# pearl-robot-lab/2HandedAfforder

Measured on AMD Instinct MI355X. Metric: affordance frames/sec/GPU @1024^2, 32-tok prompt; mask IoU vs ref, higher is better.
Workload: dtype bf16

## Files before the change

2handedafforder_amd/csrc/window_attention.hip:

```cpp
#include "haff_common.h"

namespace {

struct WinArgs {
  const bf16_t *q, *k, *v;
  bf16_t* o;
  long q_sb, q_sh, q_st;
  long k_sb, k_sh, k_st;
  long v_sb, v_sh, v_st;
  long o_sb, o_sh, o_st;
  int B, H;
  float scale;
  const bf16_t *tab_h, *tab_w;
  int grid_h, grid_w, wps;
  long pad_token;
};

constexpr float WLOG2E = 1.4426950408889634f;
typedef __attribute__((address_space(3))) bf16x4* wlds_v4_ptr;
typedef const __attribute__((address_space(1))) void* wgptr_t;
typedef __attribute__((address_space(3))) void* wlptr_t;
__device__ __attribute__((aligned(16))) unsigned int haff_win_zero_page[4];

template <int D, int S>
struct WinCfg {
  static constexpr int N = S * S;
  static constexpr int NKD = (D + 31) / 32;
  static constexpr int ND = D / 16;
  static constexpr int CPR = D / 8;
  static constexpr int KPC = (D * 2) % 64 == 32 ? 0 : 2;
  static constexpr int KSTR = D * 2 + 16 * KPC;
  static constexpr int VSTR = D * 2;
  static constexpr int NKS = (S + 1) / 2;
  static constexpr int RS = 52;
  static constexpr int QPW = 2;
  static constexpr int NWAVES = (S + QPW - 1) / QPW;
  static constexpr int NTHREADS = 64 * NWAVES;
  static constexpr int KSLOTS = N * (CPR + KPC), VSLOTS = N * CPR;
  static constexpr int K_BYTES = N * KSTR, V_BYTES = N * VSTR;
  static constexpr int PAD_SLOTS = (KSLOTS + VSLOTS + 63) / 64 * 64;
  static constexpr int BUF_BYTES = PAD_SLOTS * 16;
  static constexpr int SC_BYTES = NWAVES * 16 * RS * 4;
  static constexpr int LDS_BYTES = 2 * BUF_BYTES + SC_BYTES;
};

template <int D, int S, bool F16 = false>
__global__ __launch_bounds__((WinCfg<D, S>::NTHREADS)) void window_attn_kernel(WinArgs p) {
  using E = h16<F16>;
  using C = WinCfg<D, S>;
  static_assert(D % 16 == 0 && D <= 96 && S <= 16 && 2 * S - 1 <= 32, "window kernel geometry");
  extern __shared__ __attribute__((aligned(16))) unsigned char wsm[];
  float* sScr = reinterpret_cast<float*>(wsm + 2 * C::BUF_BYTES);

  const int tid = threadIdx.x;
  const int lane = tid & 63;
  const int wave = __builtin_amdgcn_readfirstlane(tid >> 6);
  const int fr = lane & 15, fh = lane >> 4;
  const int n_items = p.B * p.H;

  auto decode = [&](int id, int& win, int& h) {
    if ((p.B & 7) == 0) {
      const int x = id & 7, kseq = id >> 3;
      win = (kseq / p.H) * 8 + x;
      h = kseq - (kseq / p.H) * p.H;
    } else {
      win = id / p.H;
      h = id - win * p.H;
    }
  };

  constexpr int TOTAL_SLOTS = C::KSLOTS + C::VSLOTS;
  constexpr int NDMA = (C::PAD_SLOTS + C::NTHREADS - 1) / C::NTHREADS;
  static_assert((C::K_BYTES % 16) == 0 && C::KSTR == (C::CPR + C::KPC) * 16 && C::VSTR == C::CPR * 16 && C::KSTR % 64 == 32, "slot layout");
  unsigned slot_off[NDMA];
  unsigned slot_pad[NDMA];
  const long v_minus_k = (p.v - p.k);
  const unsigned vmk_bytes = (unsigned)(v_minus_k * 2);
#pragma unroll
  for (int i = 0; i < NDMA; ++i) {
    const int sl = tid + i * C::NTHREADS;
    long off;
    unsigned pad = 0;
    if (sl >= TOTAL_SLOTS) {
      off = 0;
    } else if (sl < C::KSLOTS) {
      const int row = sl / (C::CPR + C::KPC), c = sl - row * (C::CPR + C::KPC);
      off = (long)row * p.k_st + (c < C::CPR ? c * 8 : 0);
      pad = ((unsigned)(row / S) << 28) | ((unsigned)(row % S) << 24) | (unsigned)((c < C::CPR ? c : 0) * 16);
    } else {
      const int sv = sl - C::KSLOTS;
      const int row = sv / C::CPR, c = sv - row * C::CPR;
      off = v_minus_k + (long)row * p.v_st + c * 8;
      pad = ((unsigned)(row / S) << 28) | ((unsigned)(row % S) << 24) | (1u << 23) | (unsigned)(c * 16);
    }
    slot_off[i] = (unsigned)(off * 2);
    slot_pad[i] = pad;
  }
  uint4 qnext[C::QPW][C::NKD];
  const int qcol = min(fr, S - 1);
  const bf16_t* nx_kb = p.k;
  int nx_pad_h0 = S, nx_pad_w0 = S;
  unsigned nx_pad_base = 0, nx_lds0 = 0;
  auto begin_loads = [&](int id, int buf) {
    int win, h;
    decode(id, win, h);
    const bf16_t* qb = p.q + (long)win * p.q_sb + (long)h * p.q_sh;
    const bf16_t* kb = p.k + (long)win * p.k_sb + (long)h * p.k_sh;
    int pad_h0 = S, pad_w0 = S;
    if (p.grid_h > 0) {
      const int wi = win % (p.wps * p.wps);
      pad_h0 = p.grid_h - (wi / p.wps) * S;
      pad_w0 = p.grid_w - (wi % p.wps) * S;
    }
    const unsigned pad_base = (unsigned)((p.pad_token * p.k_st - (long)win * p.k_sb) * 2);
    const bf16_t* qpad = p.q + p.pad_token * p.q_st + (long)h * p.q_sh;
#pragma unroll
    for (int t = 0; t < C::QPW; ++t) {
      const int qh_t = min(wave + t * C::NWAVES, S - 1);
      const bf16_t* qsrc = (qh_t >= pad_h0 || qcol >= pad_w0) ? qpad : qb + (long)(qh_t * S + qcol) * p.q_st;
#pragma unroll
      for (int kd = 0; kd < C::NKD; ++kd) {
        const int col = kd * 32 + fh * 8;
        qnext[t][kd] = make_uint4(0, 0, 0, 0);
        if (col < D) qnext[t][kd] = *reinterpret_cast<const uint4*>(qsrc + col);
      }
    }
    nx_kb = kb;
    nx_pad_h0 = pad_h0;
    nx_pad_w0 = pad_w0;
    nx_pad_base = pad_base;
    nx_lds0 = (unsigned)(uintptr_t)(wlptr_t)(wsm + buf * C::BUF_BYTES) + wave * 1024;
  };
  auto issue_dma = [&](int i0, int i1) {
#pragma unroll
    for (int i = 0; i < NDMA; ++i) {
      if (i < i0 || i >= i1) continue;
      const unsigned m0v = nx_lds0 + i * C::NTHREADS * 16;
      const bool is_pad = (int)(slot_pad[i] >> 28) >= nx_pad_h0 || (int)((slot_pad[i] >> 24) & 15u) >= nx_pad_w0;
      const unsigned off = is_pad ? nx_pad_base + (slot_pad[i] & 0xffu) + ((slot_pad[i] >> 23) & 1u) * vmk_bytes : slot_off[i];
      if ((i + 1) * C::NTHREADS <= C::PAD_SLOTS || (i * C::NTHREADS + wave * 64) < C::PAD_SLOTS)
        asm volatile("s_mov_b32 m0, %2\n\ts_nop 0\n\tglobal_load_lds_dwordx4 %0, %1" ::"v"(off), "s"(nx_kb), "s"(m0v)
                     : "memory");
    }
  };
  constexpr int DMA_Q1 = (NDMA + 3) / 4, DMA_Q2 = (NDMA + 1) / 2, DMA_Q3 = (3 * NDMA + 3) / 4;

  auto settle_q = [&]() {
#pragma unroll
    for (int t = 0; t < C::QPW; ++t)
#pragma unroll
      for (int kd = 0; kd < C::NKD; ++kd)
        asm volatile("" : "+v"(qnext[t][kd].x), "+v"(qnext[t][kd].y), "+v"(qnext[t][kd].z), "+v"(qnext[t][kd].w));
  };

  int item = blockIdx.x;
  if (item >= n_items) return;
  begin_loads(item, 0);
  issue_dma(0, NDMA);

  bf16x8 th[2][C::NKD], tw[2][C::NKD];
#pragma unroll
  for (int mt = 0; mt < 2; ++mt) {
    const int r = min(mt * 16 + fr, 2 * S - 2);
#pragma unroll
    for (int kd = 0; kd < C::NKD; ++kd) {
      const int col = kd * 32 + fh * 8;
      uint4 a = make_uint4(0, 0, 0, 0), b = make_uint4(0, 0, 0, 0);
      if (col < D) {
        a = *reinterpret_cast<const uint4*>(p.tab_h + r * D + col);
        b = *reinterpret_cast<const uint4*>(p.tab_w + r * D + col);
      }
      th[mt][kd] = __builtin_bit_cast(bf16x8, a);
      tw[mt][kd] = __builtin_bit_cast(bf16x8, b);
    }
  }
  asm volatile("s_waitcnt vmcnt(0)" ::: "memory");
  settle_q();
#pragma unroll
  for (int mt = 0; mt < 2; ++mt)
#pragma unroll
    for (int kd = 0; kd < C::NKD; ++kd) {
      asm volatile("" : "+v"(th[mt][kd]));
      asm volatile("" : "+v"(tw[mt][kd]));
    }
  __syncthreads();

  const float sl2 = p.scale * WLOG2E;
  float* scr = sScr + wave * (16 * C::RS);
  const int tr_q = fr >> 2, tr_p = fr & 3;
  bool kw_ok[4];
#pragma unroll
  for (int j = 0; j < 4; ++j) kw_ok[j] = (4 * fh + j) < S;

  for (int it = 0;; ++it) {
    const int buf = it & 1;
    const unsigned char* sK = wsm + buf * C::BUF_BYTES;
    const unsigned char* sV = sK + C::K_BYTES;
    int win, h;
    decode(item, win, h);
    bf16_t* ob = p.o + (long)win * p.o_sb + (long)h * p.o_sh;
    uint4 qcur[C::QPW][C::NKD];
#pragma unroll
    for (int t = 0; t < C::QPW; ++t)
#pragma unroll
      for (int kd = 0; kd < C::NKD; ++kd) qcur[t][kd] = qnext[t][kd];
    const int next = item + gridDim.x;
    const bool has_next = next < n_items;
    if (has_next) {
      begin_loads(next, buf ^ 1);
      issue_dma(0, DMA_Q1);
    }

#pragma unroll
    for (int t = 0; t < C::QPW; ++t) {
      const int qh = wave + t * C::NWAVES;
      static_assert(C::QPW * C::NWAVES == S, "q-tiles must divide evenly over the waves");
      bf16x8 qraw[C::NKD], qs[C::NKD];
#pragma unroll
      for (int kd = 0; kd < C::NKD; ++kd) {
        const uint4 r = qcur[t][kd];
        uint4 rs = make_uint4(0, 0, 0, 0);
        if (kd * 32 + fh * 8 < D) {
          float qv[8];
          const unsigned w4[4] = {r.x, r.y, r.z, r.w};
#pragma unroll
          for (int j = 0; j < 4; ++j) {
            qv[2 * j] = E::lo(w4[j]) * sl2;
            qv[2 * j + 1] = E::hi(w4[j]) * sl2;
          }
          rs.x = E::pack2(qv[0], qv[1]); rs.y = E::pack2(qv[2], qv[3]);
          rs.z = E::pack2(qv[4], qv[5]); rs.w = E::pack2(qv[6], qv[7]);
        }
        qraw[kd] = __builtin_bit_cast(bf16x8, r);
        qs[kd] = __builtin_bit_cast(bf16x8, rs);
      }

      float relw4[4], relh_t[S];
      {
        f32x4 t0 = f32x4{0.f, 0.f, 0.f, 0.f}, t1 = t0;
#pragma unroll
        for (int kd = 0; kd < C::NKD; ++kd) {
          t0 = E::mfma16(tw[0][kd], qraw[kd], t0);
          t1 = E::mfma16(tw[1][kd], qraw[kd], t1);
        }
        float a[4] = {t0[0], t0[1], t0[2], t0[3]}, b[4] = {t1[0], t1[1], t1[2], t1[3]};
        store4(scr + fr * C::RS + 4 * fh, a);
        store4(scr + fr * C::RS + 16 + 4 * fh, b);
        __builtin_amdgcn_wave_barrier();
#pragma unroll
        for (int j = 0; j < 4; ++j) {
          const int r = min(max(qcol - (4 * fh + j) + S - 1, 0), 2 * S - 2);
          relw4[j] = kw_ok[j] ? scr[fr * C::RS + r] * WLOG2E : -INFINITY;
        }
        __builtin_amdgcn_wave_barrier();
      }
      {
        f32x4 t0 = f32x4{0.f, 0.f, 0.f, 0.f}, t1 = t0;
#pragma unroll
        for (int kd = 0; kd < C::NKD; ++kd) {
          t0 = E::mfma16(th[0][kd], qraw[kd], t0);
          t1 = E::mfma16(th[1][kd], qraw[kd], t1);
        }
        float a[4] = {t0[0], t0[1], t0[2], t0[3]}, b[4] = {t1[0], t1[1], t1[2], t1[3]};
        store4(scr + fr * C::RS + 4 * fh, a);
        store4(scr + fr * C::RS + 16 + 4 * fh, b);
        __builtin_amdgcn_wave_barrier();
#pragma unroll
        for (int kt = 0; kt < S; ++kt) relh_t[kt] = scr[fr * C::RS + (qh - kt + S - 1)] * WLOG2E;
        __builtin_amdgcn_wave_barrier();
      }

      f32x4 sacc[S];
#pragma unroll
      for (int kt = 0; kt < S; ++kt)
        sacc[kt] = f32x4{relw4[0] + relh_t[kt], relw4[1] + relh_t[kt], relw4[2] + relh_t[kt], relw4[3] + relh_t[kt]};
      constexpr int KG = (S + 1) / 2;
      const int koff_last = (D * 2 - (C::NKD - 1) * 64 == 32) ? (C::NKD - 1) * 64 - 32 + ((fh + 2) & 3) * 16
                                                              : min(fh * 16 + (C::NKD - 1) * 64, D * 2 - 16);
#pragma unroll
      for (int g0 = 0; g0 < S; g0 += KG) {
#pragma unroll
        for (int kd = 0; kd < C::NKD; ++kd) {
#pragma unroll
          for (int kt = g0; kt < g0 + KG && kt < S; ++kt) {
            const bf16x8 kf = *reinterpret_cast<const bf16x8*>(sK + (kt * S + qcol) * C::KSTR + (kd == C::NKD - 1 ? koff_last : fh * 16 + kd * 64));
            sacc[kt] = E::mfma16(kf, qs[kd], sacc[kt]);
          }
        }
        __builtin_amdgcn_sched_barrier(0);
      }

      if (has_next) {
        if (t == 0) issue_dma(DMA_Q1, DMA_Q2);
        else issue_dma(DMA_Q3, NDMA);
      }
      float mx = -1e30f;
#pragma unroll
      for (int kt = 0; kt < S; ++kt)
#pragma unroll
        for (int j = 0; j < 4; ++j) mx = fmaxf(mx, sacc[kt][j]);
      mx = fmaxf(mx, __shfl_xor(mx, 16, 64));
      mx = fmaxf(mx, __shfl_xor(mx, 32, 64));
      float psum = 0.f;
#pragma unroll
      for (int kt = 0; kt < S; ++kt)
#pragma unroll
        for (int j = 0; j < 4; ++j) {
          const float e = __builtin_amdgcn_exp2f(sacc[kt][j] - mx);
          sacc[kt][j] = e;
          psum += e;
        }
      psum += __shfl_xor(psum, 16, 64);
      psum += __shfl_xor(psum, 32, 64);

      f32x4 oacc[C::ND];
#pragma unroll
      for (int dt = 0; dt < C::ND; ++dt) oacc[dt] = f32x4{0.f, 0.f, 0.f, 0.f};
      const int vkw = min(4 * fh + tr_q, S - 1);
#pragma unroll
      for (int ks = 0; ks < C::NKS; ++ks) {
        constexpr int dummy = 0; (void)dummy;
        const int t0 = 2 * ks, t1 = (2 * ks + 1 < S) ? 2 * ks + 1 : 2 * ks;
        uint4 u;
        u.x = E::pack2(sacc[t0][0], sacc[t0][1]);
        u.y = E::pack2(sacc[t0][2], sacc[t0][3]);
        u.z = (2 * ks + 1 < S) ? E::pack2(sacc[t1][0], sacc[t1][1]) : 0u;
        u.w = (2 * ks + 1 < S) ? E::pack2(sacc[t1][2], sacc[t1][3]) : 0u;
        const bf16x8 pf = __builtin_bit_cast(bf16x8, u);
        const unsigned char* v0 = sV + (t0 * S + vkw) * C::VSTR + 8 * tr_p;
        const unsigned char* v1 = sV + (t1 * S + vkw) * C::VSTR + 8 * tr_p;
#pragma unroll
        for (int dt = 0; dt < C::ND; ++dt) {
          const bf16x4 lo = __builtin_amdgcn_ds_read_tr16_b64_v4i16((wlds_v4_ptr)(v0 + 32 * dt));
          const bf16x4 hi = __builtin_amdgcn_ds_read_tr16_b64_v4i16((wlds_v4_ptr)(v1 + 32 * dt));
          const bf16x8 vf = __builtin_shufflevector(lo, hi, 0, 1, 2, 3, 4, 5, 6, 7);
          oacc[dt] = E::mfma16(vf, pf, oacc[dt]);
        }
      }

      if (has_next && t == 0) issue_dma(DMA_Q2, DMA_Q3);
      const float inv = 1.0f / psum;
      if (fr < S) {
        bf16_t* orow = ob + (long)(qh * S + fr) * p.o_st + 4 * fh;
#pragma unroll
        for (int dt = 0; dt < C::ND; ++dt) {
          float v[4] = {oacc[dt][0] * inv, oacc[dt][1] * inv, oacc[dt][2] * inv, oacc[dt][3] * inv};
          store4h<F16>(orow + 16 * dt, v);
        }
      }
    }

    if (!has_next) break;
    item = next;
    asm volatile("s_waitcnt vmcnt(0)" ::: "memory");
    settle_q();
    __syncthreads();
  }
}

}

template <bool F16 = false>
static int window_attention_impl(const void* q, long q_sb, long q_sh, long q_st,
                                 const void* k, long k_sb, long k_sh, long k_st,
                                 const void* v, long v_sb, long v_sh, long v_st,
                                 void* o, long o_sb, long o_sh, long o_st,
                                 int n_windows, int H, int S, int d, float scale,
                                 const void* tab_h, const void* tab_w, int grid_h, int grid_w,
                                 long pad_token, void* stream) {
  if (n_windows <= 0 || H <= 0 || S <= 0 || d <= 0 || !tab_h || !tab_w) return HAFF_ERR_BAD_ARG;
  if ((q_st & 7) || (k_st & 7) || (v_st & 7) || (o_st & 3) || (q_sh & 7) || (k_sh & 7) || (v_sh & 7) || (o_sh & 3) ||
      (q_sb & 7) || (k_sb & 7) || (v_sb & 7) || (o_sb & 3))
    return HAFF_ERR_BAD_ARG;
  if ((reinterpret_cast<uintptr_t>(q) & 15) || (reinterpret_cast<uintptr_t>(k) & 15) ||
      (reinterpret_cast<uintptr_t>(v) & 15) || (reinterpret_cast<uintptr_t>(o) & 7) ||
      (reinterpret_cast<uintptr_t>(tab_h) & 15) || (reinterpret_cast<uintptr_t>(tab_w) & 15))
    return HAFF_ERR_BAD_ARG;
  if (S != 14 || d != 80) return HAFF_ERR_UNSUPPORTED;
  if (k_sb != v_sb || k_sh != v_sh || k_st != v_st) return HAFF_ERR_UNSUPPORTED;
  {
    const long dvk = reinterpret_cast<const bf16_t*>(v) - reinterpret_cast<const bf16_t*>(k);
    const long span = (dvk < 0 ? -dvk : dvk) + (long)S * S * k_st + d;
    if (dvk < 0 || span * 2 >= (1L << 32)) return HAFF_ERR_UNSUPPORTED;
  }
  WinArgs p{reinterpret_cast<const bf16_t*>(q), reinterpret_cast<const bf16_t*>(k), reinterpret_cast<const bf16_t*>(v),
            reinterpret_cast<bf16_t*>(o), q_sb, q_sh, q_st, k_sb, k_sh, k_st, v_sb, v_sh, v_st, o_sb, o_sh, o_st,
            n_windows, H, scale, reinterpret_cast<const bf16_t*>(tab_h), reinterpret_cast<const bf16_t*>(tab_w),
            grid_h, grid_w, grid_h > 0 ? (grid_h + S - 1) / S : 0, pad_token};
  if (grid_h > 0) {
    if (grid_w != grid_h || (n_windows % (p.wps * p.wps)) != 0 || pad_token < 0 || q_st != k_st ||
        (pad_token + 1) * k_st * 2 >= (1L << 32) || pad_token * k_st < (long)(n_windows - 1) * k_sb)
      return HAFF_ERR_BAD_ARG;
    const long dvk = reinterpret_cast<const bf16_t*>(v) - reinterpret_cast<const bf16_t*>(k);
    if ((pad_token * k_st + dvk + d) * 2 >= (1L << 32)) return HAFF_ERR_UNSUPPORTED;
  }
  using C = WinCfg<80, 14>;
  if (hipFuncSetAttribute(reinterpret_cast<const void*>(&window_attn_kernel<80, 14, F16>),
                          hipFuncAttributeMaxDynamicSharedMemorySize, C::LDS_BYTES) != hipSuccess)
    return HAFF_ERR_LAUNCH;
  const int n_items = n_windows * H;
  dim3 grid(n_items < 256 ? n_items : 256), block(C::NTHREADS);
  hipLaunchKernelGGL((window_attn_kernel<80, 14, F16>), grid, block, C::LDS_BYTES, reinterpret_cast<hipStream_t>(stream), p);
  return haff_check_launch();
}

extern "C" int haff_window_attention_bf16(const void* q, long q_sb, long q_sh, long q_st,
                                          const void* k, long k_sb, long k_sh, long k_st,
                                          const void* v, long v_sb, long v_sh, long v_st,
                                          void* o, long o_sb, long o_sh, long o_st,
                                          int n_windows, int H, int S, int d, float scale,
                                          const void* tab_h, const void* tab_w, int grid_h, int grid_w,
                                          long pad_token, void* stream) {
  return window_attention_impl(q, q_sb, q_sh, q_st, k, k_sb, k_sh, k_st, v, v_sb, v_sh, v_st, o, o_sb, o_sh, o_st, n_windows, H, S,
                               d, scale, tab_h, tab_w, grid_h, grid_w, pad_token, stream);
}

extern "C" int haff_window_attention_f16(const void* q, long q_sb, long q_sh, long q_st,
                                         const void* k, long k_sb, long k_sh, long k_st,
                                         const void* v, long v_sb, long v_sh, long v_st,
                                         void* o, long o_sb, long o_sh, long o_st,
                                         int n_windows, int H, int S, int d, float scale,
                                         const void* tab_h, const void* tab_w, int grid_h, int grid_w,
                                         long pad_token, void* stream) {
  return window_attention_impl<true>(q, q_sb, q_sh, q_st, k, k_sb, k_sh, k_st, v, v_sb, v_sh, v_st, o, o_sb, o_sh, o_st, n_windows, H,
                                     S, d, scale, tab_h, tab_w, grid_h, grid_w, pad_token, stream);
}
```

Baseline: 114.1.

## Interleave both query tiles per wave and move rel-pos tables to LDS

Processes both query rows of each wave together, so every K and V LDS fragment read is reused across two MFMAs and one rel-pos table fragment feeds both tiles. The relative-position tables move from per-thread registers into LDS, written once by wave 0. Slot pad metadata is now recomputed only for edge windows instead of being kept in registers, and the Q prefetch is deferred to after softmax. The aim is lower register pressure and fewer LDS reads per MFMA, at the cost of larger live accumulator arrays (two sets of sacc and oacc), extra LDS reads for the table fragments, and a different DMA issue schedule.

```diff
diff --git a/2handedafforder_amd/csrc/window_attention.hip b/2handedafforder_amd/csrc/window_attention.hip
--- a/2handedafforder_amd/csrc/window_attention.hip
+++ b/2handedafforder_amd/csrc/window_attention.hip
@@ -41,7 +41,8 @@
   static constexpr int PAD_SLOTS = (KSLOTS + VSLOTS + 63) / 64 * 64;
   static constexpr int BUF_BYTES = PAD_SLOTS * 16;
   static constexpr int SC_BYTES = NWAVES * 16 * RS * 4;
-  static constexpr int LDS_BYTES = 2 * BUF_BYTES + SC_BYTES;
+  static constexpr int TAB_BYTES = 2 * 2 * NKD * 64 * 16;
+  static constexpr int LDS_BYTES = 2 * BUF_BYTES + SC_BYTES + TAB_BYTES;
 };
 
 template <int D, int S, bool F16 = false>
@@ -51,6 +52,7 @@
   static_assert(D % 16 == 0 && D <= 96 && S <= 16 && 2 * S - 1 <= 32, "window kernel geometry");
   extern __shared__ __attribute__((aligned(16))) unsigned char wsm[];
   float* sScr = reinterpret_cast<float*>(wsm + 2 * C::BUF_BYTES);
+  unsigned char* sTab = wsm + 2 * C::BUF_BYTES + C::SC_BYTES;
 
   const int tid = threadIdx.x;
   const int lane = tid & 63;
@@ -72,33 +74,37 @@
   constexpr int TOTAL_SLOTS = C::KSLOTS + C::VSLOTS;
   constexpr int NDMA = (C::PAD_SLOTS + C::NTHREADS - 1) / C::NTHREADS;
   static_assert((C::K_BYTES % 16) == 0 && C::KSTR == (C::CPR + C::KPC) * 16 && C::VSTR == C::CPR * 16 && C::KSTR % 64 == 32, "slot layout");
-  unsigned slot_off[NDMA];
-  unsigned slot_pad[NDMA];
   const long v_minus_k = (p.v - p.k);
   const unsigned vmk_bytes = (unsigned)(v_minus_k * 2);
+  auto slot_pad = [&](int sl) -> unsigned {
+    if (sl >= TOTAL_SLOTS) return 0u;
+    if (sl < C::KSLOTS) {
+      const int row = sl / (C::CPR + C::KPC), c = sl - row * (C::CPR + C::KPC);
+      return ((unsigned)(row / S) << 28) | ((unsigned)(row % S) << 24) | (unsigned)((c < C::CPR ? c : 0) * 16);
+    }
+    const int sv = sl - C::KSLOTS;
+    const int row = sv / C::CPR, c = sv - row * C::CPR;
+    return ((unsigned)(row / S) << 28) | ((unsigned)(row % S) << 24) | (1u << 23) | (unsigned)(c * 16);
+  };
+  unsigned slot_off[NDMA];
 #pragma unroll
   for (int i = 0; i < NDMA; ++i) {
     const int sl = tid + i * C::NTHREADS;
-    long off;
-    unsigned pad = 0;
-    if (sl >= TOTAL_SLOTS) {
-      off = 0;
-    } else if (sl < C::KSLOTS) {
+    long off = 0;
+    if (sl < C::KSLOTS) {
       const int row = sl / (C::CPR + C::KPC), c = sl - row * (C::CPR + C::KPC);
       off = (long)row * p.k_st + (c < C::CPR ? c * 8 : 0);
-      pad = ((unsigned)(row / S) << 28) | ((unsigned)(row % S) << 24) | (unsigned)((c < C::CPR ? c : 0) * 16);
-    } else {
+    } else if (sl < TOTAL_SLOTS) {
       const int sv = sl - C::KSLOTS;
       const int row = sv / C::CPR, c = sv - row * C::CPR;
       off = v_minus_k + (long)row * p.v_st + c * 8;
-      pad = ((unsigned)(row / S) << 28) | ((unsigned)(row % S) << 24) | (1u << 23) | (unsigned)(c * 16);
     }
     slot_off[i] = (unsigned)(off * 2);
-    slot_pad[i] = pad;
   }
   uint4 qnext[C::QPW][C::NKD];
   const int qcol = min(fr, S - 1);
   const bf16_t* nx_kb = p.k;
+  const bf16_t* nx_q[C::QPW];
   int nx_pad_h0 = S, nx_pad_w0 = S;
   unsigned nx_pad_base = 0, nx_lds0 = 0;
   auto begin_loads = [&](int id, int buf) {
@@ -117,13 +123,7 @@
 #pragma unroll
     for (int t = 0; t < C::QPW; ++t) {
       const int qh_t = min(wave + t * C::NWAVES, S - 1);
-      const bf16_t* qsrc = (qh_t >= pad_h0 || qcol >= pad_w0) ? qpad : qb + (long)(qh_t * S + qcol) * p.q_st;
-#pragma unroll
-      for (int kd = 0; kd < C::NKD; ++kd) {
-        const int col = kd * 32 + fh * 8;
-        qnext[t][kd] = make_uint4(0, 0, 0, 0);
-        if (col < D) qnext[t][kd] = *reinterpret_cast<const uint4*>(qsrc + col);
-      }
+      nx_q[t] = (qh_t >= pad_h0 || qcol >= pad_w0) ? qpad : qb + (long)(qh_t * S + qcol) * p.q_st;
     }
     nx_kb = kb;
     nx_pad_h0 = pad_h0;
@@ -131,13 +131,26 @@
     nx_pad_base = pad_base;
     nx_lds0 = (unsigned)(uintptr_t)(wlptr_t)(wsm + buf * C::BUF_BYTES) + wave * 1024;
   };
+  auto load_q = [&]() {
+#pragma unroll
+    for (int t = 0; t < C::QPW; ++t)
+#pragma unroll
+      for (int kd = 0; kd < C::NKD; ++kd)
+        qnext[t][kd] = *reinterpret_cast<const uint4*>(nx_q[t] + min(kd * 32 + fh * 8, D - 8));
+  };
   auto issue_dma = [&](int i0, int i1) {
 #pragma unroll
     for (int i = 0; i < NDMA; ++i) {
       if (i < i0 || i >= i1) continue;
       const unsigned m0v = nx_lds0 + i * C::NTHREADS * 16;
-      const bool is_pad = (int)(slot_pad[i] >> 28) >= nx_pad_h0 || (int)((slot_pad[i] >> 24) & 15u) >= nx_pad_w0;
-      const unsigned off = is_pad ? nx_pad_base + (slot_pad[i] & 0xffu) + ((slot_pad[i] >> 23) & 1u) * vmk_bytes : slot_off[i];
+      unsigned off = slot_off[i];
+      if (nx_pad_h0 < S || nx_pad_w0 < S) {
+        int t_id = tid;
+        asm volatile("" : "+v"(t_id));
+        const unsigned sp = slot_pad(t_id + i * C::NTHREADS);
+        if ((int)(sp >> 28) >= nx_pad_h0 || (int)((sp >> 24) & 15u) >= nx_pad_w0)
+          off = nx_pad_base + (sp & 0xffu) + ((sp >> 23) & 1u) * vmk_bytes;
+      }
       if ((i + 1) * C::NTHREADS <= C::PAD_SLOTS || (i * C::NTHREADS + wave * 64) < C::PAD_SLOTS)
         asm volatile("s_mov_b32 m0, %2\n\ts_nop 0\n\tglobal_load_lds_dwordx4 %0, %1" ::"v"(off), "s"(nx_kb), "s"(m0v)
                      : "memory");
@@ -156,33 +169,40 @@
   int item = blockIdx.x;
   if (item >= n_items) return;
   begin_loads(item, 0);
+  load_q();
   issue_dma(0, NDMA);
 
-  bf16x8 th[2][C::NKD], tw[2][C::NKD];
-#pragma unroll
-  for (int mt = 0; mt < 2; ++mt) {
-    const int r = min(mt * 16 + fr, 2 * S - 2);
-#pragma unroll
-    for (int kd = 0; kd < C::NKD; ++kd) {
-      const int col = kd * 32 + fh * 8;
-      uint4 a = make_uint4(0, 0, 0, 0), b = make_uint4(0, 0, 0, 0);
-      if (col < D) {
-        a = *reinterpret_cast<const uint4*>(p.tab_h + r * D + col);
-        b = *reinterpret_cast<const uint4*>(p.tab_w + r * D + col);
-      }
-      th[mt][kd] = __builtin_bit_cast(bf16x8, a);
-      tw[mt][kd] = __builtin_bit_cast(bf16x8, b);
-    }
+  auto tab_frag = [&](int tab, int mt, int kd) -> unsigned char* {
+    return sTab + ((tab * 2 + mt) * C::NKD + kd) * 1024 + lane * 16;
+  };
+  if (wave == 0) {
+    uint4 tv[2][2][C::NKD];
+#pragma unroll
+    for (int mt = 0; mt < 2; ++mt) {
+      const int r = min(mt * 16 + fr, 2 * S - 2);
+#pragma unroll
+      for (int kd = 0; kd < C::NKD; ++kd) {
+        const int col = kd * 32 + fh * 8;
+        tv[0][mt][kd] = tv[1][mt][kd] = make_uint4(0, 0, 0, 0);
+        if (col < D) {
+          tv[0][mt][kd] = *reinterpret_cast<const uint4*>(p.tab_h + r * D + col);
+          tv[1][mt][kd] = *reinterpret_cast<const uint4*>(p.tab_w + r * D + col);
+        }
+      }
+    }
+    asm volatile("s_waitcnt vmcnt(0)" ::: "memory");
+#pragma unroll
+    for (int tb = 0; tb < 2; ++tb)
+#pragma unroll
+      for (int mt = 0; mt < 2; ++mt)
+#pragma unroll
+        for (int kd = 0; kd < C::NKD; ++kd) {
+          asm volatile("" : "+v"(tv[tb][mt][kd].x), "+v"(tv[tb][mt][kd].y), "+v"(tv[tb][mt][kd].z), "+v"(tv[tb][mt][kd].w));
+          *reinterpret_cast<uint4*>(tab_frag(tb, mt, kd)) = tv[tb][mt][kd];
+        }
   }
   asm volatile("s_waitcnt vmcnt(0)" ::: "memory");
   settle_q();
-#pragma unroll
-  for (int mt = 0; mt < 2; ++mt)
-#pragma unroll
-    for (int kd = 0; kd < C::NKD; ++kd) {
-      asm volatile("" : "+v"(th[mt][kd]));
-      asm volatile("" : "+v"(tw[mt][kd]));
-    }
   __syncthreads();
 
   const float sl2 = p.scale * WLOG2E;
@@ -199,6 +219,7 @@
     int win, h;
     decode(item, win, h);
     bf16_t* ob = p.o + (long)win * p.o_sb + (long)h * p.o_sh;
+    settle_q();
     uint4 qcur[C::QPW][C::NKD];
 #pragma unroll
     for (int t = 0; t < C::QPW; ++t)
@@ -211,16 +232,17 @@
       issue_dma(0, DMA_Q1);
     }
 
-#pragma unroll
-    for (int t = 0; t < C::QPW; ++t) {
-      const int qh = wave + t * C::NWAVES;
-      static_assert(C::QPW * C::NWAVES == S, "q-tiles must divide evenly over the waves");
-      bf16x8 qraw[C::NKD], qs[C::NKD];
+    static_assert(C::QPW * C::NWAVES == S, "q-tiles must divide evenly over the waves");
+    constexpr int T = C::QPW;
+    bf16x8 qraw[T][C::NKD], qs[T][C::NKD];
+#pragma unroll
+    for (int t = 0; t < T; ++t)
 #pragma unroll
       for (int kd = 0; kd < C::NKD; ++kd) {
-        const uint4 r = qcur[t][kd];
+        const bool in_d = kd * 32 + fh * 8 < D;
+        const uint4 r = in_d ? qcur[t][kd] : make_uint4(0, 0, 0, 0);
         uint4 rs = make_uint4(0, 0, 0, 0);
-        if (kd * 32 + fh * 8 < D) {
+        if (in_d) {
           float qv[8];
           const unsigned w4[4] = {r.x, r.y, r.z, r.w};
 #pragma unroll
@@ -231,120 +253,140 @@
           rs.x = E::pack2(qv[0], qv[1]); rs.y = E::pack2(qv[2], qv[3]);
           rs.z = E::pack2(qv[4], qv[5]); rs.w = E::pack2(qv[6], qv[7]);
         }
-        qraw[kd] = __builtin_bit_cast(bf16x8, r);
-        qs[kd] = __builtin_bit_cast(bf16x8, rs);
-      }
-
-      float relw4[4], relh_t[S];
-      {
-        f32x4 t0 = f32x4{0.f, 0.f, 0.f, 0.f}, t1 = t0;
-#pragma unroll
-        for (int kd = 0; kd < C::NKD; ++kd) {
-          t0 = E::mfma16(tw[0][kd], qraw[kd], t0);
-          t1 = E::mfma16(tw[1][kd], qraw[kd], t1);
-        }
-        float a[4] = {t0[0], t0[1], t0[2], t0[3]}, b[4] = {t1[0], t1[1], t1[2], t1[3]};
+        qraw[t][kd] = __builtin_bit_cast(bf16x8, r);
+        qs[t][kd] = __builtin_bit_cast(bf16x8, rs);
+      }
+
+    float relw4[T][4], relh_t[T][S];
+#pragma unroll
+    for (int tb = 1; tb >= 0; --tb) {
+      f32x4 ta[T][2];
+#pragma unroll
+      for (int t = 0; t < T; ++t) ta[t][0] = ta[t][1] = f32x4{0.f, 0.f, 0.f, 0.f};
+#pragma unroll
+      for (int kd = 0; kd < C::NKD; ++kd) {
+        const bf16x8 f0 = *reinterpret_cast<const bf16x8*>(tab_frag(tb, 0, kd));
+        const bf16x8 f1 = *reinterpret_cast<const bf16x8*>(tab_frag(tb, 1, kd));
+#pragma unroll
+        for (int t = 0; t < T; ++t) {
+          ta[t][0] = E::mfma16(f0, qraw[t][kd], ta[t][0]);
+          ta[t][1] = E::mfma16(f1, qraw[t][kd], ta[t][1]);
+        }
+      }
+#pragma unroll
+      for (int t = 0; t < T; ++t) {
+        float a[4] = {ta[t][0][0], ta[t][0][1], ta[t][0][2], ta[t][0][3]}, b[4] = {ta[t][1][0], ta[t][1][1], ta[t][1][2], ta[t][1][3]};
         store4(scr + fr * C::RS + 4 * fh, a);
         store4(scr + fr * C::RS + 16 + 4 * fh, b);
         __builtin_amdgcn_wave_barrier();
-#pragma unroll
-        for (int j = 0; j < 4; ++j) {
-          const int r = min(max(qcol - (4 * fh + j) + S - 1, 0), 2 * S - 2);
-          relw4[j] = kw_ok[j] ? scr[fr * C::RS + r] * WLOG2E : -INFINITY;
+        if (tb == 1) {
+#pragma unroll
+          for (int j = 0; j < 4; ++j) {
+            const int r = min(max(qcol - (4 * fh + j) + S - 1, 0), 2 * S - 2);
+            relw4[t][j] = kw_ok[j] ? scr[fr * C::RS + r] * WLOG2E : -INFINITY;
+          }
+        } else {
+          const int qh = wave + t * C::NWAVES;
+#pragma unroll
+          for (int kt = 0; kt < S; ++kt) relh_t[t][kt] = scr[fr * C::RS + (qh - kt + S - 1)] * WLOG2E;
         }
         __builtin_amdgcn_wave_barrier();
       }
-      {
-        f32x4 t0 = f32x4{0.f, 0.f, 0.f, 0.f}, t1 = t0;
-#pragma unroll
-        for (int kd = 0; kd < C::NKD; ++kd) {
-          t0 = E::mfma16(th[0][kd], qraw[kd], t0);
-          t1 = E::mfma16(th[1][kd], qraw[kd], t1);
-        }
-        float a[4] = {t0[0], t0[1], t0[2], t0[3]}, b[4] = {t1[0], t1[1], t1[2], t1[3]};
-        store4(scr + fr * C::RS + 4 * fh, a);
-        store4(scr + fr * C::RS + 16 + 4 * fh, b);
-        __builtin_amdgcn_wave_barrier();
-#pragma unroll
-        for (int kt = 0; kt < S; ++kt) relh_t[kt] = scr[fr * C::RS + (qh - kt + S - 1)] * WLOG2E;
-        __builtin_amdgcn_wave_barrier();
-      }
-
-      f32x4 sacc[S];
+    }
+
+    f32x4 sacc[T][S];
+#pragma unroll
+    for (int t = 0; t < T; ++t)
 #pragma unroll
       for (int kt = 0; kt < S; ++kt)
-        sacc[kt] = f32x4{relw4[0] + relh_t[kt], relw4[1] + relh_t[kt], relw4[2] + relh_t[kt], relw4[3] + relh_t[kt]};
-      constexpr int KG = (S + 1) / 2;
-      const int koff_last = (D * 2 - (C::NKD - 1) * 64 == 32) ? (C::NKD - 1) * 64 - 32 + ((fh + 2) & 3) * 16
-                                                              : min(fh * 16 + (C::NKD - 1) * 64, D * 2 - 16);
-#pragma unroll
-      for (int g0 = 0; g0 < S; g0 += KG) {
-#pragma unroll
-        for (int kd = 0; kd < C::NKD; ++kd) {
-#pragma unroll
-          for (int kt = g0; kt < g0 + KG && kt < S; ++kt) {
-            const bf16x8 kf = *reinterpret_cast<const bf16x8*>(sK + (kt * S + qcol) * C::KSTR + (kd == C::NKD - 1 ? koff_last : fh * 16 + kd * 64));
-            sacc[kt] = E::mfma16(kf, qs[kd], sacc[kt]);
-          }
-        }
-        __builtin_amdgcn_sched_barrier(0);
-      }
-
-      if (has_next) {
-        if (t == 0) issue_dma(DMA_Q1, DMA_Q2);
-        else issue_dma(DMA_Q3, NDMA);
-      }
+        sacc[t][kt] = f32x4{relw4[t][0] + relh_t[t][kt], relw4[t][1] + relh_t[t][kt], relw4[t][2] + relh_t[t][kt],
+                            relw4[t][3] + relh_t[t][kt]};
+    constexpr int KG = (S + 3) / 4;
+    const int koff_last = (D * 2 - (C::NKD - 1) * 64 == 32) ? (C::NKD - 1) * 64 - 32 + ((fh + 2) & 3) * 16
+                                                            : min(fh * 16 + (C::NKD - 1) * 64, D * 2 - 16);
+#pragma unroll
+    for (int g0 = 0; g0 < S; g0 += KG) {
+#pragma unroll
+      for (int kd = 0; kd < C::NKD; ++kd) {
+#pragma unroll
+        for (int kt = g0; kt < g0 + KG && kt < S; ++kt) {
+          const bf16x8 kf = *reinterpret_cast<const bf16x8*>(sK + (kt * S + qcol) * C::KSTR + (kd == C::NKD - 1 ? koff_last : fh * 16 + kd * 64));
+#pragma unroll
+          for (int t = 0; t < T; ++t) sacc[t][kt] = E::mfma16(kf, qs[t][kd], sacc[t][kt]);
+        }
+      }
+      __builtin_amdgcn_sched_barrier(0);
+      if (has_next && g0 == 0) issue_dma(DMA_Q1, DMA_Q2);
+    }
+    if (has_next) issue_dma(DMA_Q2, DMA_Q3);
+
+    float psum[T];
+    bf16x8 pf[T][C::NKS];
+#pragma unroll
+    for (int t = 0; t < T; ++t) {
       float mx = -1e30f;
 #pragma unroll
       for (int kt = 0; kt < S; ++kt)
 #pragma unroll
-        for (int j = 0; j < 4; ++j) mx = fmaxf(mx, sacc[kt][j]);
+        for (int j = 0; j < 4; ++j) mx = fmaxf(mx, sacc[t][kt][j]);
       mx = fmaxf(mx, __shfl_xor(mx, 16, 64));
       mx = fmaxf(mx, __shfl_xor(mx, 32, 64));
-      float psum = 0.f;
+      float ps = 0.f;
 #pragma unroll
       for (int kt = 0; kt < S; ++kt)
 #pragma unroll
         for (int j = 0; j < 4; ++j) {
-          const float e = __builtin_amdgcn_exp2f(sacc[kt][j] - mx);
-          sacc[kt][j] = e;
-          psum += e;
-        }
-      psum += __shfl_xor(psum, 16, 64);
-      psum += __shfl_xor(psum, 32, 64);
-
-      f32x4 oacc[C::ND];
-#pragma unroll
-      for (int dt = 0; dt < C::ND; ++dt) oacc[dt] = f32x4{0.f, 0.f, 0.f, 0.f};
-      const int vkw = min(4 * fh + tr_q, S - 1);
+          const float e = __builtin_amdgcn_exp2f(sacc[t][kt][j] - mx);
+          sacc[t][kt][j] = e;
+          ps += e;
+        }
+      ps += __shfl_xor(ps, 16, 64);
+      ps += __shfl_xor(ps, 32, 64);
+      psum[t] = ps;
 #pragma unroll
       for (int ks = 0; ks < C::NKS; ++ks) {
-        constexpr int dummy = 0; (void)dummy;
         const int t0 = 2 * ks, t1 = (2 * ks + 1 < S) ? 2 * ks + 1 : 2 * ks;
         uint4 u;
-        u.x = E::pack2(sacc[t0][0], sacc[t0][1]);
-        u.y = E::pack2(sacc[t0][2], sacc[t0][3]);
-        u.z = (2 * ks + 1 < S) ? E::pack2(sacc[t1][0], sacc[t1][1]) : 0u;
-        u.w = (2 * ks + 1 < S) ? E::pack2(sacc[t1][2], sacc[t1][3]) : 0u;
-        const bf16x8 pf = __builtin_bit_cast(bf16x8, u);
-        const unsigned char* v0 = sV + (t0 * S + vkw) * C::VSTR + 8 * tr_p;
-        const unsigned char* v1 = sV + (t1 * S + vkw) * C::VSTR + 8 * tr_p;
-#pragma unroll
-        for (int dt = 0; dt < C::ND; ++dt) {
-          const bf16x4 lo = __builtin_amdgcn_ds_read_tr16_b64_v4i16((wlds_v4_ptr)(v0 + 32 * dt));
-          const bf16x4 hi = __builtin_amdgcn_ds_read_tr16_b64_v4i16((wlds_v4_ptr)(v1 + 32 * dt));
-          const bf16x8 vf = __builtin_shufflevector(lo, hi, 0, 1, 2, 3, 4, 5, 6, 7);
-          oacc[dt] = E::mfma16(vf, pf, oacc[dt]);
-        }
-      }
-
-      if (has_next && t == 0) issue_dma(DMA_Q2, DMA_Q3);
-      const float inv = 1.0f / psum;
+        u.x = E::pack2(sacc[t][t0][0], sacc[t][t0][1]);
+        u.y = E::pack2(sacc[t][t0][2], sacc[t][t0][3]);
+        u.z = (2 * ks + 1 < S) ? E::pack2(sacc[t][t1][0], sacc[t][t1][1]) : 0u;
+        u.w = (2 * ks + 1 < S) ? E::pack2(sacc[t][t1][2], sacc[t][t1][3]) : 0u;
+        pf[t][ks] = __builtin_bit_cast(bf16x8, u);
+      }
+    }
+    load_q();
+    if (has_next) issue_dma(DMA_Q3, NDMA);
+
+    f32x4 oacc[T][C::ND];
+#pragma unroll
+    for (int t = 0; t < T; ++t)
+#pragma unroll
+      for (int dt = 0; dt < C::ND; ++dt) oacc[t][dt] = f32x4{0.f, 0.f, 0.f, 0.f};
+    const int vkw = min(4 * fh + tr_q, S - 1);
+#pragma unroll
+    for (int ks = 0; ks < C::NKS; ++ks) {
+      const int t0 = 2 * ks, t1 = (2 * ks + 1 < S) ? 2 * ks + 1 : 2 * ks;
+      const unsigned char* v0 = sV + (t0 * S + vkw) * C::VSTR + 8 * tr_p;
+      const unsigned char* v1 = sV + (t1 * S + vkw) * C::VSTR + 8 * tr_p;
+#pragma unroll
+      for (int dt = 0; dt < C::ND; ++dt) {
+        const bf16x4 lo = __builtin_amdgcn_ds_read_tr16_b64_v4i16((wlds_v4_ptr)(v0 + 32 * dt));
+        const bf16x4 hi = __builtin_amdgcn_ds_read_tr16_b64_v4i16((wlds_v4_ptr)(v1 + 32 * dt));
+        const bf16x8 vf = __builtin_shufflevector(lo, hi, 0, 1, 2, 3, 4, 5, 6, 7);
+#pragma unroll
+        for (int t = 0; t < T; ++t) oacc[t][dt] = E::mfma16(vf, pf[t][ks], oacc[t][dt]);
+      }
+    }
+
+#pragma unroll
+    for (int t = 0; t < T; ++t) {
+      const float inv = 1.0f / psum[t];
+      const int qh = wave + t * C::NWAVES;
       if (fr < S) {
         bf16_t* orow = ob + (long)(qh * S + fr) * p.o_st + 4 * fh;
 #pragma unroll
         for (int dt = 0; dt < C::ND; ++dt) {
-          float v[4] = {oacc[dt][0] * inv, oacc[dt][1] * inv, oacc[dt][2] * inv, oacc[dt][3] * inv};
+          float v[4] = {oacc[t][dt][0] * inv, oacc[t][dt][1] * inv, oacc[t][dt][2] * inv, oacc[t][dt][3] * inv};
           store4h<F16>(orow + 16 * dt, v);
         }
       }
```

Result: no change. 113.9, median of 2 (-0.1%).
